# ParBLiSS/kmerhash

Measured on AMD Instinct MI355X. Metric: kmer_inserts_plus_finds_per_sec, higher is better.
Workload: dtype u64

## Files before the change

kmerhash_amd/csrc/kh_kernels.h:

```cpp
#pragma once
#include <hip/hip_runtime.h>
#include <stdint.h>
#include "../../include/kmerhash_amd/kh_hash.h"

#define KH_LB 11
#define KH_L (1u << KH_LB)
#define KH_HS 4096u
#define KH_CHUNK_THREADS 512
#ifndef KH_PART_THREADS
#define KH_PART_THREADS 512
#define KH_PART_MAXPER 4
#endif
#ifndef KH_PART_ITEMS
#define KH_PART_ITEMS 16
#endif
#define KH_PART_TILE (KH_PART_THREADS * KH_PART_ITEMS)
#ifndef KH_PART_STAGE
#define KH_PART_STAGE 4096
#endif
#define KH_NONE 0xFFFFFFFFFFFFFFFFull
#define KH_EMPTY_KEY 0xFFFFFFFFFFFFFFFFull

enum { KHK_RH = 0, KHK_LP = 1 };
enum { KH_FLAG_PROBE_OVERFLOW = 0, KH_FLAG_REGION_OVERFLOW = 1, KH_FLAG_COUNT_OVERFLOW = 2, KH_FLAG_INTERNAL = 3, KH_FLAG_FUSE_INVALID = 4, KH_NFLAGS = 8 };
// ... 777 lines not shown
      const unsigned long long iv = ((unsigned long long)i << 32) | (vbase ? *reinterpret_cast<const uint32_t*>(vbase + i * vstride) : vconst);
      orec[(uint64_t)q * n + pos] = make_ulonglong2(key, iv);
    }
  }
  __syncthreads();
  if (tid == 0) { cursor[q] = (uint64_t)q * n + cnt; starts[q] = (uint64_t)q * n; if (q == 0) starts[gridDim.x] = (uint64_t)gridDim.x * n; }
}

#define KH_SAMPLE_N 65536u
#define KH_SAMPLE_SET (1u << 18)
__global__ void k_sample_dups(const char* __restrict__ kbase, uint32_t kstride, uint64_t n, unsigned long long* __restrict__ set ,
                              uint32_t* __restrict__ dups) {
  const uint32_t i = blockIdx.x * blockDim.x + threadIdx.x;
  if (i >= KH_SAMPLE_N) return;
  const uint64_t pos = (uint64_t)i * (n / KH_SAMPLE_N);
  const unsigned long long key = *reinterpret_cast<const uint64_t*>(kbase + pos * kstride) ^ 0x8000000000000001ull;
  const unsigned long long tag = key ? key : 1ull;
  uint32_t slot = (uint32_t)kh_fmix64(tag) & (KH_SAMPLE_SET - 1);
  for (;;) {
    const unsigned long long cur = atomicCAS(&set[slot], 0ull, tag);
    if (cur == 0ull) break;
    if (cur == tag) { atomicAdd(dups, 1u); break; }
    slot = (slot + 1) & (KH_SAMPLE_SET - 1);
  }
}

__global__ void k_init_cursors2(unsigned long long* __restrict__ cur1, uint64_t n1, uint64_t slot1, unsigned long long* __restrict__ cur2,
                                uint64_t* __restrict__ starts, uint64_t n2, uint64_t slot2, uint32_t* __restrict__ ovf) {
  const uint64_t i = (uint64_t)blockIdx.x * blockDim.x + threadIdx.x;
  if (i < n1) cur1[i] = i * slot1;
  if (i < n2) cur2[i] = i * slot2;
  if (i <= n2) starts[i] = i * slot2;
  if (i == 0) *ovf = 0u;
}
__global__ void k_init_cursors(unsigned long long* __restrict__ cursor, uint64_t* __restrict__ starts, uint64_t n, uint64_t slot) {
  const uint64_t i = (uint64_t)blockIdx.x * blockDim.x + threadIdx.x;
  if (i < n) cursor[i] = i * slot;
  if (starts && i <= n) starts[i] = i * slot;
}

__global__ void k_make_tiles(const uint64_t* __restrict__ segoff, uint32_t nseg, KhTile* __restrict__ tiles, uint32_t* __restrict__ ntiles_out,
                             const unsigned long long* __restrict__ cursor = nullptr, uint64_t slot = 0) {
  __shared__ uint32_t wtot[16];
  __shared__ uint32_t carry_s;
  const uint32_t tid = threadIdx.x, lane = tid & 63, wid = tid >> 6;
  if (tid == 0) carry_s = 0;
  __syncthreads();
  for (uint32_t base = 0; base < nseg; base += 1024) {
    uint32_t s = base + tid;
    uint64_t beg = 0, len = 0;
    if (s < nseg) {
      if (slot) { beg = (uint64_t)s * slot; len = cursor[s] - beg; if (len > slot) len = slot; }
      else { beg = segoff[s]; len = segoff[s + 1] - beg; }
    }
    uint32_t nt = (uint32_t)((len + KH_PART_TILE - 1) / KH_PART_TILE);
    uint32_t incl = nt;
    for (int off = 1; off < 64; off <<= 1) {
      uint32_t o = __shfl_up(incl, off, 64);
      if (lane >= (uint32_t)off) incl += o;
    }
    if (lane == 63) wtot[wid] = incl;
    __syncthreads();
    uint32_t wpre = 0;
    for (uint32_t w = 0; w < wid; ++w) wpre += wtot[w];
    uint32_t carry = carry_s;
    uint32_t first = carry + wpre + incl - nt;
// ... 633 lines not shown
    KhMP v; v.A = KH_MP_NEG; v.n = 0;
#pragma unroll
    for (int j = 0; j < KH_CARRY_ITEMS; ++j) {
      it[j].A = KH_MP_NEG; it[j].n = 0;
      if (c0 + j < nch) { it[j].A = sumA[c0 + j]; it[j].n = sumN[c0 + j]; }
      v = kh_mp_combine(v, it[j]);
    }
    KhMP total;
    KhMP excl = kh_block_scan_mp(v, s_wtot, &total);
    const KhMP carry = s_carry;
    KhMP run = kh_mp_combine(carry, excl);
#pragma unroll
    for (int j = 0; j < KH_CARRY_ITEMS; ++j) {
      if (c0 + j < nch) prefix_tmp[c0 + j] = run;
      run = kh_mp_combine(run, it[j]);
    }
    __syncthreads();
    if (tid == 0) s_carry = kh_mp_combine(carry, total);
    __syncthreads();
  }
  KhMP all = s_carry;
  long long end0 = all.A > all.n ? all.A : all.n;
  long long x0 = end0 - cap;
  if (x0 < 0) x0 = 0;
  for (uint32_t c = tid; c < nch; c += 1024) {
    KhMP p = prefix_tmp[c];
    long long x = x0 + p.n;
    xcarry[c] = p.A > x ? p.A : x;
  }
}

#define KH_SPILL 256
template <int KIND, int HASH>
__global__ __launch_bounds__(KH_CHUNK_THREADS) void k_chunk_place(KhRebuildParams P) {
  __shared__ uint64_t skeys[KH_L + KH_SPILL];
  __shared__ uint32_t svals[KH_L + KH_SPILL];
  __shared__ uint32_t sinfo_w[(KH_L + KH_SPILL) / 4];
  __shared__ uint32_t fill[KH_L];
  __shared__ uint32_t start[KH_L];
  __shared__ uint32_t s_emin;
  __shared__ long long s_pend;
  __shared__ KhMP s_wtot[KH_CHUNK_THREADS / 64];
  uint8_t* sinfo = reinterpret_cast<uint8_t*>(sinfo_w);
  const uint32_t tid = threadIdx.x, c = blockIdx.x;
  const uint32_t Ln = P.New.cap > KH_L ? KH_L : (uint32_t)P.New.cap;
  const uint64_t Sc = (uint64_t)c * Ln, mask_n = P.New.cap - 1;
  const uint32_t empty4 = KIND == KHK_RH ? 0u : 0x40404040u;
  for (uint32_t i = tid; i < KH_L + KH_SPILL; i += KH_CHUNK_THREADS) { skeys[i] = 0; svals[i] = 0; }
  for (uint32_t i = tid; i < (KH_L + KH_SPILL) / 4; i += KH_CHUNK_THREADS) sinfo_w[i] = empty4;
  uint32_t cb[KH_HOMES_PER_THREAD];
  KhMP v; v.A = KH_MP_NEG; v.n = 0;
#pragma unroll
  for (uint32_t j = 0; j < KH_HOMES_PER_THREAD; ++j) {
    uint32_t b = tid * KH_HOMES_PER_THREAD + j;
    cb[j] = b < Ln ? P.homecnt[Sc + b] : 0u;
    if (b < Ln) { KhMP h; h.A = (long long)b + cb[j]; h.n = cb[j]; v = kh_mp_combine(v, h); }
    fill[tid * KH_HOMES_PER_THREAD + j] = 0;
  }
  KhMP excl = kh_block_scan_mp(v, s_wtot, nullptr);
  const long long xr = P.xcarry[c] - (long long)Sc;
  long long p = excl.A > xr + excl.n ? excl.A : xr + excl.n;
#pragma unroll
  for (uint32_t j = 0; j < KH_HOMES_PER_THREAD; ++j) {
    uint32_t b = tid * KH_HOMES_PER_THREAD + j;
    if (b < Ln) {
      long long st = p > (long long)b ? p : (long long)b;
      start[b] = (uint32_t)st;
      p = st + cb[j];
    }
  }
  if (tid == KH_CHUNK_THREADS - 1) s_pend = p;
  __syncthreads();
  auto place = [&](uint64_t key, uint32_t val, uint64_t hn) {
    uint32_t b = (uint32_t)(hn - Sc);
    uint32_t r = atomicAdd(&fill[b], 1u);
    uint32_t prel = start[b] + r;
    uint32_t dist = prel - b;
    uint8_t ib = 0x00;
    if (KIND == KHK_RH) {
      if (dist > 127u) { atomicOr(&P.flags[KH_FLAG_PROBE_OVERFLOW], 1u); dist = 127u; }
      ib = (uint8_t)(0x80u | dist);
    }
    if (prel < KH_L + KH_SPILL) { skeys[prel] = key; svals[prel] = val; sinfo[prel] = ib; }
    else kh_slot_st(P.New.s + ((Sc + prel) & mask_n), key, val, ib);
  };
  kh_for_each_old<KIND, HASH>(P, c, &s_emin, place);
  kh_for_each_new<HASH>(P, c, place);
  __syncthreads();
  long long pend = s_pend;
  if (pend < (long long)Ln) pend = Ln;
  const uint32_t lo = xr > 0 ? (uint32_t)xr : 0u;
  uint32_t hi = pend < (long long)(KH_L + KH_SPILL) ? (uint32_t)pend : (KH_L + KH_SPILL);
  for (uint32_t s0 = lo + tid; s0 < hi; s0 += KH_CHUNK_THREADS) {
    kh_slot_st(P.New.s + ((Sc + s0) & mask_n), skeys[s0], svals[s0], sinfo[s0]);
  }
}

#define KH_XB 127u
#define KH_FSPILL 128u
struct KhFusedParams {
  KhSrcSet src; uint32_t PB;
  KhSlots New; KhSeed seed; int mode;
  unsigned long long* pub;
  uint64_t* ck0; uint32_t* cv0; uint16_t* homecnt0;
  uint32_t* maxidx;
  uint64_t n_total, half_max_load;
  uint64_t base_size;
  unsigned long long* est;
  uint32_t* flags;
  long long poll_limit;
  int nodup;
  KhRebuildParams R;
};

template <int KIND, int HASH, bool MERGE>
__device__ __forceinline__ uint32_t kh_stage_from_table(const KhRebuildParams& R, uint32_t c, uint64_t Sc, unsigned long long* lk,
                                                         unsigned long long* liv, uint32_t* n_staged, uint32_t* scratch) {
  const uint32_t tid = threadIdx.x;
  const uint64_t cap_o = R.Old.cap, mask_o = cap_o - 1, mask_n = R.New.cap - 1;
  if (tid == 0) *n_staged = 0;
  __syncthreads();
  if (cap_o) {
    const uint32_t nch_o = (uint32_t)(cap_o >> KH_LB);
    const uint32_t o = c & (nch_o - 1);
    const bool same = R.New.cap == cap_o;
    const uint64_t S = (uint64_t)o * KH_L;
    uint64_t len = KH_L + 128u;
    if (KIND == KHK_LP) {
      const uint64_t beyond = cap_o - KH_L;
// ... 1234 lines not shown
    if ((late >> k) & 1u) {
      const uint32_t p0 = pj[k] & 0xFFFFu, pc = (pj[k] >> 16) + xr;
      enter(kh_slot_key(w[k]), w[k].z, rank[k] >> 16, p0 > pc ? p0 : pc);
    }
  }
#pragma unroll
  for (uint32_t u = 0; u < 2; ++u) {
    if ((late >> (ROWS + u)) & 1u) {
      const uint32_t i = tid + u * KH_CHUNK_THREADS;
      const uint32_t p0 = pj[ROWS + u] & 0xFFFFu, pc = (pj[ROWS + u] >> 16) + xr;
      enter(rk[i], (uint32_t)riv[i], hbr[u], p0 > pc ? p0 : pc);
    }
  }
  __syncthreads();
  {
    const int tA = total.A > 0 ? total.A : 0;
    int pend = tA > (int)xr + (int)n_c ? tA : (int)xr + (int)n_c;
    if (pend < (int)KH_L) pend = (int)KH_L;
    if (pend > (int)(KH_L + KH_FSPILL)) pend = (int)(KH_L + KH_FSPILL);
#pragma unroll
    for (uint32_t k = 0; k < ROWS; ++k) {
      const int s0 = (int)(base + 64u * k);
      if (k < nrows && s0 >= (int)xr && s0 < pend) {
        const uint32_t ib = iinfo[s0];
        KhSlot* dst = P.New.s + ((Sc + (uint32_t)s0) & mask_n);
        if (ib == 0u) kh_slot_st(dst, 0, 0, kh_empty_info<KHK_RH>());
        else kh_slot_st(dst, ikey[s0], ival[s0], ib);
      }
    }
  }
  (void)n_old;
}

__global__ void k_fused_tail_carry(const unsigned long long* __restrict__ pub, uint32_t nch, long long* __restrict__ xcarry0,
                                   uint64_t* __restrict__ noff0 = nullptr, uint32_t* __restrict__ ncnt0 = nullptr) {
  if (threadIdx.x == 0 && blockIdx.x == 0) {
    xcarry0[0] = (long long)((pub[nch - 1] >> 32) & 0x7FFFFFFFull);
    if (noff0) { noff0[0] = 0; noff0[1] = 0; }
    if (ncnt0) ncnt0[0] = (uint32_t)pub[0];
  }
}

__global__ __launch_bounds__(1024) void k_fused_totals(const unsigned long long* __restrict__ pub, const uint32_t* __restrict__ maxidx, uint32_t nch,
                                                       unsigned long long* __restrict__ totals) {
  __shared__ unsigned long long ws[16];
  __shared__ uint32_t wm[16];
  unsigned long long sum = 0; uint32_t mx = 0;
  for (uint32_t c = blockIdx.x * 1024 + threadIdx.x; c < nch; c += gridDim.x * 1024) { sum += pub[c] & 0xFFFFFFFFull; const uint32_t v = maxidx[c]; mx = v > mx ? v : mx; }
  for (int off = 32; off > 0; off >>= 1) { sum += __shfl_down(sum, off, 64); const uint32_t o = __shfl_down(mx, off, 64); mx = o > mx ? o : mx; }
  if ((threadIdx.x & 63) == 0) { ws[threadIdx.x >> 6] = sum; wm[threadIdx.x >> 6] = mx; }
  __syncthreads();
  if (threadIdx.x == 0) {
    unsigned long long t = 0; uint32_t m = 0;
    for (int w = 0; w < 16; ++w) { t += ws[w]; m = wm[w] > m ? wm[w] : m; }
    if (t) atomicAdd(&totals[0], t);
    if (m) atomicMax(&totals[1], (unsigned long long)m);
  }
}

__global__ void k_disp_hist(const KhSlot* __restrict__ slots, uint64_t cap, unsigned long long* __restrict__ out128) {
  __shared__ uint32_t h[128];
  if (threadIdx.x < 128) h[threadIdx.x] = 0;
  __syncthreads();
  uint64_t i = (uint64_t)blockIdx.x * blockDim.x + threadIdx.x;
  uint64_t stride = (uint64_t)gridDim.x * blockDim.x;
  for (; i < cap; i += stride) { uint32_t b = slots[i].info & 0xFFu; if (b >= 0x80u) atomicAdd(&h[b & 0x7Fu], 1u); }
  __syncthreads();
  if (threadIdx.x < 128 && h[threadIdx.x]) atomicAdd(&out128[threadIdx.x], (unsigned long long)h[threadIdx.x]);
}

template <int KIND>
__global__ void k_unpack_slots(const KhSlot* __restrict__ slots, uint64_t cap, uint64_t* __restrict__ keys, uint32_t* __restrict__ vals,
                               uint8_t* __restrict__ info, uint8_t* __restrict__ flags) {
  uint64_t i = (uint64_t)blockIdx.x * blockDim.x + threadIdx.x;
  uint64_t stride = (uint64_t)gridDim.x * blockDim.x;
  for (; i < cap; i += stride) {
    const uint4 w = kh_slot_ld(slots + i);
    if (keys) keys[i] = kh_slot_key(w);
    if (vals) vals[i] = w.z;
    if (info) info[i] = (uint8_t)(w.w & 0xFFu);
    if (flags) flags[i] = kh_is_occupied<KIND>(w.w & 0xFFu) ? 1 : 0;
  }
}

#define KH_SHARD_THREADS 512
#define KH_SHARD_TILE(KW) (KH_SHARD_THREADS * KhKey<KW>::SHARD_ITEMS)
#define KH_SHARD_MAXR 64
// ... 676 lines not shown
```

kmerhash_amd/csrc/kmerhash_amd.hip:

```cpp
#include "kh_kernels.h"
#include "kh_kernels_wide.h"
#include "kh_kernels_values.h"
#include "kh_kernels_index.h"
#include "kh_kernels_index_wide.h"
#include "kh_kernels_csr.h"
#include "../../include/kmerhash_amd.h"

#include <string>
#include <vector>
#include <cstdio>
#include <cstring>
#include <algorithm>
#include <cmath>
#include <cstdlib>

#include <map>
#include <memory>
#include <mutex>
#include <unordered_map>

#define KH_VERSION_STR "kmerhash_amd 0.1 (gfx950)"

namespace {
struct DevPool {
// ... 47 lines not shown
  P.free_.insert(std::make_pair(it->second, p));
  P.cached += it->second;
}
struct HostPool { std::mutex m; std::vector<uint64_t*> pinned; std::vector<hipEvent_t> events[16]; };
HostPool g_host;
uint64_t* pinned_get() {
  { std::lock_guard<std::mutex> g(g_host.m);
    if (!g_host.pinned.empty()) { uint64_t* p = g_host.pinned.back(); g_host.pinned.pop_back(); return p; } }
  uint64_t* p = nullptr;
  if (hipHostMalloc(reinterpret_cast<void**>(&p), 64 * sizeof(uint64_t)) != hipSuccess) { (void)hipGetLastError(); return nullptr; }
  return p;
}
void pinned_put(uint64_t* p) { if (p) { std::lock_guard<std::mutex> g(g_host.m); g_host.pinned.push_back(p); } }
hipEvent_t event_get(int dev) {
  { std::lock_guard<std::mutex> g(g_host.m);
    auto& v = g_host.events[dev & 15];
    if (!v.empty()) { hipEvent_t e = v.back(); v.pop_back(); return e; } }
  hipEvent_t e = nullptr;
  hipEventCreate(&e);
  return e;
}
void event_put(int dev, hipEvent_t e) { if (e) { std::lock_guard<std::mutex> g(g_host.m); g_host.events[dev & 15].push_back(e); } }
}

namespace {

struct ProfRec { const char* name; hipEvent_t a, b; };

struct Block { char* p; size_t cap; };

}

struct SlackShared { unsigned long long* cur2; uint64_t* starts; uint32_t* ovf; uint64_t slot; };
struct SlotBuf {
  void* p; uint64_t cap;
  SlotBuf() : p(nullptr), cap(0) {}
  SlotBuf(KhSlots s) : p(s.s), cap(s.cap) {}
  SlotBuf(KwSlots s) : p(s.s), cap(s.cap) {}
};
struct kh_table {
  int kind = KHK_RH, hash = 0, device = 0;
  KhSeed seed = KhSeed{0, 0u};
  hipStream_t stream = nullptr;
  float min_lf = 0.f, max_lf = 0.f;
  uint64_t min_load = 0, max_load = 0, lsize = 0;
  uint32_t slot_bytes = sizeof(KhSlot);
  SlotBuf cur, spare;
  std::vector<Block> blocks;
  size_t blk = 0, off = 0;
  uint64_t* hpin = nullptr;
  std::string err;
  struct {
    bool active, fallback, nodup; int mode;
    bool repeatable, slack, rec12;
    SlackShared sh;
    uint64_t n_total, fed, cap_u; uint32_t PB;
    ulonglong2 *tmp, *fin;
    KhSrcSet S;
    uint64_t* stage_k; uint32_t* stage_v;
    const uint64_t* wk[KH_MAX_SRC]; const uint32_t* wv[KH_MAX_SRC]; uint64_t wn[KH_MAX_SRC]; uint32_t wsrc; uint32_t* wcnt;
  } ins = {};
  uint32_t* part_overflow = nullptr;
  double batch_vf = 1.0;
  bool batch_nodup = false;
  bool prof = false;
  std::vector<ProfRec> recs;
  std::vector<std::pair<std::string, std::pair<double, uint64_t> > > prof_acc;
};
struct kh_wtable : kh_table {};

namespace {

inline uint64_t next_pow2(uint64_t x) {
  if (x <= 1) return 1;
  return uint64_t(1) << (64 - __builtin_clzll(x - 1));
}
inline uint64_t threshold(uint64_t buckets, float lf) {
  return static_cast<uint64_t>(static_cast<float>(buckets) * lf);
}
inline uint32_t log2u(uint64_t x) { return 63u - (uint32_t)__builtin_clzll(x); }

kh_status fail(kh_table* t, kh_status s, const std::string& msg) {
  if (t) t->err = msg;
  return s;
}
#define HIPCHK(call)                                                                                   \
  do {                                                                                                 \
    hipError_t e__ = (call);                                                                           \
    if (e__ != hipSuccess)                                                                             \
      return fail(t, e__ == hipErrorOutOfMemory ? KH_ERR_NOMEM : KH_ERR_HIP,                          \
                  std::string(#call) + ": " + hipGetErrorString(e__));                                \
  } while (0)

void arena_reset(kh_table* t) { t->blk = 0; t->off = 0; }
kh_status arena_take(kh_table* t, size_t bytes, void** out) {
// ... 129 lines not shown
  if ((k) == KHK_RH) { constexpr int KIND = KHK_RH; KH_SWITCH_HASH(h, __VA_ARGS__) }  \
  else { constexpr int KIND = KHK_LP; KH_SWITCH_HASH(h, __VA_ARGS__) }

inline uint32_t grid_for(uint64_t n, uint32_t block, uint32_t maxblocks = 256 * 16) {
  uint64_t g = (n + block - 1) / block;
  if (g < 1) g = 1;
  if (g > maxblocks) g = maxblocks;
  return (uint32_t)g;
}

template <typename T>
kh_status stage_in(kh_table* t, const void* p, uint64_t n, kh_mem where, const T** out) {
  if (where == KH_MEM_DEVICE || p == nullptr) { *out = static_cast<const T*>(p); return KH_OK; }
  T* d = nullptr;
  TAKE(d, T, n);
  HIPCHK(hipMemcpyAsync(d, p, sizeof(T) * n, hipMemcpyHostToDevice, t->stream));
  *out = d;
  return KH_OK;
}

inline size_t ws_rebuild(uint64_t cap) { return size_t(cap) * 2 + (cap > KH_L ? (cap >> KH_LB) : 1) * 48 + (size_t(1) << 16); }

struct PreCount { uint16_t* homecnt; long long* sumA; long long* sumN; };

const bool g_disable_fused_rebuild = getenv("KH_DISABLE_FUSED_BUILD") != nullptr || getenv("KH_DISABLE_FUSED_REBUILD") != nullptr;

const long long g_poll_limit = getenv("KH_DEBUG_POLL_LIMIT") ? atoll(getenv("KH_DEBUG_POLL_LIMIT")) : (1ll << 23);
struct FusedRun { unsigned long long* totals; uint32_t* flags; };
const bool g_disable_lean = getenv("KH_DISABLE_LEAN_BUILD") != nullptr;
kh_status launch_fused(kh_table* t, int src, KhFusedParams& F, const KhSlots& nw, uint32_t PB_tail, const char* name, FusedRun* out) {
  const uint32_t nch = (uint32_t)(nw.cap >> KH_LB);
  char* blk; uint32_t* maxidx; uint64_t* ck0; uint32_t* cv0; uint16_t* hc0; long long* xc0; uint64_t* noff0; uint32_t* ncnt0;
  const size_t sz_pub = (size_t)nch * 8, sz_ctl = sz_pub + 256, sz_all = sz_ctl + (size_t)nch * 4;
  TAKE(blk, char, sz_all);
  maxidx = reinterpret_cast<uint32_t*>(blk + sz_ctl);
  TAKE(ck0, uint64_t, KH_DD_M); TAKE(cv0, uint32_t, KH_DD_M); TAKE(hc0, uint16_t, KH_L); TAKE(xc0, long long, 1);
  TAKE(noff0, uint64_t, 2); TAKE(ncnt0, uint32_t, 1);
  HIPCHK(hipMemsetAsync(blk, 0, sz_all, t->stream));
  F.New = nw; F.seed = t->seed;
  F.pub = reinterpret_cast<unsigned long long*>(blk);
  unsigned long long* totals = reinterpret_cast<unsigned long long*>(blk + sz_pub);
  F.maxidx = maxidx; F.ck0 = ck0; F.cv0 = cv0; F.homecnt0 = hc0;
  F.est = reinterpret_cast<unsigned long long*>(blk + sz_pub + 32);
  F.flags = reinterpret_cast<uint32_t*>(blk + sz_pub + 64);
  F.poll_limit = g_poll_limit;
  F.R.New = nw; F.R.seed = t->seed; F.R.flags = F.flags;
  { Launch L(t, name);
    const double mean_c = (double)F.n_total / (double)nch;
    const bool lean_fits = mean_c + 5.0 * std::sqrt(mean_c) < (double)KH_LEAN_M;
    if (src == 0 && F.nodup && F.src.rec12 == 1 && F.src.n == 1 && lean_fits && !g_disable_lean) { KH_SWITCH_KIND_HASH(t->kind, t->hash, hipLaunchKernelGGL((k_build_lean<KIND, HASH>), dim3(nch), dim3(KH_CHUNK_THREADS), 0, t->stream, F)); }
    else if (src == 0) { KH_SWITCH_KIND_HASH(t->kind, t->hash, hipLaunchKernelGGL((k_build_fused<KIND, HASH, 0>), dim3(nch), dim3(KH_CHUNK_THREADS), 0, t->stream, F)); }
    else if (src == 1) { KH_SWITCH_KIND_HASH(t->kind, t->hash, hipLaunchKernelGGL((k_build_fused<KIND, HASH, 1>), dim3(nch), dim3(KH_CHUNK_THREADS), 0, t->stream, F)); }
    else if (src == 3) { KH_SWITCH_HASH(t->hash, hipLaunchKernelGGL((k_build_fused<KHK_RH, HASH, 3>), dim3(nch), dim3(KH_CHUNK_THREADS), 0, t->stream, F)); }
    else if (src == 4) { KH_SWITCH_HASH(t->hash, hipLaunchKernelGGL((k_erase_stream<HASH>), dim3(nch), dim3(KH_CHUNK_THREADS), 0, t->stream, F)); }
    else if (src == 5) { KH_SWITCH_HASH(t->hash, hipLaunchKernelGGL((k_insert_stream<HASH>), dim3(nch), dim3(KH_CHUNK_THREADS), 0, t->stream, F)); }
    else { KH_SWITCH_KIND_HASH(t->kind, t->hash, hipLaunchKernelGGL((k_build_fused<KIND, HASH, 2>), dim3(nch), dim3(KH_CHUNK_THREADS), 0, t->stream, F)); } }
  { Launch L(t, "k_fused_totals");
    hipLaunchKernelGGL(k_fused_totals, dim3(std::max<uint32_t>(1u, std::min<uint32_t>(64u, nch / 1024u))), dim3(1024), 0, t->stream, F.pub, maxidx, nch, totals); }
  {
    Launch L(t, "k_fused_tail");
    hipLaunchKernelGGL(k_fused_tail_carry, dim3(1), dim3(64), 0, t->stream, F.pub, nch, xc0, noff0, ncnt0);
    KhRebuildParams T0;
    memset(&T0, 0, sizeof(T0));
    T0.Old = kNoSlots; T0.New = nw; T0.ck = ck0; T0.cv = cv0; T0.noff = noff0; T0.ncnt = ncnt0; T0.PB = PB_tail;
    T0.seed = t->seed; T0.homecnt = hc0; T0.xcarry = xc0; T0.flags = F.flags;
    KH_SWITCH_KIND_HASH(t->kind, t->hash, hipLaunchKernelGGL((k_chunk_place<KIND, HASH>), dim3(1), dim3(KH_CHUNK_THREADS), 0, t->stream, T0));
  }
  HIPCHK(hipGetLastError());
  HIPCHK(hipMemcpyAsync(t->hpin, blk + sz_pub, 128, hipMemcpyDeviceToHost, t->stream));
  t->hpin[30] = 0;
  if (t->part_overflow) HIPCHK(hipMemcpyAsync(t->hpin + 30, t->part_overflow, 4, hipMemcpyDeviceToHost, t->stream));
  HIPCHK(hipStreamSynchronize(t->stream));
  out->totals = totals; out->flags = F.flags;
  return KH_OK;
}

const char* const kProbeOverflowText = "Robin Hood probe distance would exceed 127 (7-bit info field, hashmap_robinhood.hpp:142-144,556)";
const char* const kDedupOverflowText = "internal: de-duplication set overflow";
kh_status flags_status(kh_table* t, const uint32_t* f) {
  if (f[KH_FLAG_PROBE_OVERFLOW]) return fail(t, KH_ERR_PROBE_OVERFLOW, kProbeOverflowText);
  if (f[KH_FLAG_REGION_OVERFLOW]) return fail(t, KH_ERR_PROBE_OVERFLOW, "cluster longer than one chunk (2048 slots) without an empty slot");
  if (f[KH_FLAG_COUNT_OVERFLOW]) return fail(t, KH_ERR_PROBE_OVERFLOW, "more than 65535 keys share one home bucket");
  if (f[KH_FLAG_INTERNAL]) return fail(t, KH_ERR_HIP, kDedupOverflowText);
  return KH_OK;
}

struct Narrow {
  typedef KhSlots Slots; typedef KhRebuildParams Params;
  static Slots view(const SlotBuf& b) { return narrow(b); }
  static void set_seed(Params& P, const kh_table* t) { P.seed = t->seed; }
  static void count(kh_table* t, uint32_t nch, const Params& P) {
    Launch L(t, "k_chunk_count");
    KH_SWITCH_KIND_HASH(t->kind, t->hash, hipLaunchKernelGGL((k_chunk_count<KIND, HASH>), dim3(nch), dim3(KH_CHUNK_THREADS), 0, t->stream, P));
  }
  static void place(kh_table* t, uint32_t nch, const Params& P) {
    Launch L(t, "k_chunk_place");
    KH_SWITCH_KIND_HASH(t->kind, t->hash, hipLaunchKernelGGL((k_chunk_place<KIND, HASH>), dim3(nch), dim3(KH_CHUNK_THREADS), 0, t->stream, P));
  }
};
struct Wide {
  typedef KwSlots Slots; typedef KwRebuildParams Params;
  static Slots view(const SlotBuf& b) { return wide(b); }
  static void set_seed(Params& P, const kh_table* t) { P.seed = t->seed.s; }
  static void count(kh_table* t, uint32_t nch, const Params& P) {
// ... 94 lines not shown
    n = rh_rehash_capacity(n, t->lsize, t->max_lf);
    if (n == t->cur.cap) return KH_OK;
  } else if (t->lsize > n) {
    return fail(t, KH_ERR_FULL, "ERROR: did not find any place to insert.  should not have happend (hashmap_linearprobe.hpp:408)");
  }
  { kh_status ps = arena_prepare(t, ws_rebuild(n)); if (ps != KH_OK) return ps; }
  return rebuild(t, n, nullptr, nullptr, nullptr, nullptr, 0, false, t->lsize);
}
kh_status do_reserve(kh_table* t, uint64_t n) {
  if (n > t->max_load) return do_rehash(t, static_cast<uint64_t>(static_cast<float>(n) / t->max_lf));
  return KH_OK;
}

struct Partitioned {
  ulonglong2* rec;
  uint64_t* part_off;
  uint32_t PB, nparts;
  ulonglong2* spare;
  uint64_t slot;
  const unsigned long long* cursor;
  uint32_t* overflow;
  int rec12;
};
inline uint64_t slack_slot(double mean, double vf = 1.0) { return (uint64_t)(mean + 7.0 * std::sqrt(mean * vf) + 16.0); }
const bool g_disable_slack = getenv("KH_DISABLE_SLACK_PARTITION") != nullptr;
const int g_xcd_swizzle = getenv("KH_DISABLE_XCD_SWIZZLE") ? 0 : 1;
inline uint64_t part_buffer_records(uint64_t n, uint32_t PB, bool allow_slack, double vf = 1.0) {
  if (!allow_slack || g_disable_slack || PB <= 11 || n < (uint64_t(256) << PB)) return n;
  return (slack_slot((double)n / (double)(uint64_t(1) << PB), vf) << PB) + KH_PART_TILE;
}

kh_status partition_batch(kh_table* t, const char* kbase, uint32_t kstride, const char* vbase, uint32_t vstride,
                          uint32_t vconst, uint64_t n, uint64_t idx_base, uint32_t PB, ulonglong2* tmp, ulonglong2* fin, Partitioned& out,
                          bool allow_slack = false, int rec12 = 0, const SlackShared* shared = nullptr, bool force_slack = false, double vf = 1.0) {
  const uint32_t nparts = 1u << PB;
  out.slot = 0; out.cursor = nullptr; out.overflow = nullptr; out.rec12 = 0;
  if (shared || force_slack || part_buffer_records(n, PB, allow_slack, vf) != n) {
    const uint32_t B1 = (PB + 1) / 2, B2 = PB - B1, nb1 = 1u << B1, nb2 = 1u << B2;
    const uint64_t slot = shared ? shared->slot : slack_slot((double)n / (double)nparts, vf);
    const uint64_t slot1 = shared ? slack_slot((double)n / (double)nb1) : slot * nb2;
    unsigned long long *cur1, *cur2; uint64_t* starts; uint32_t* ovf;
    TAKE(cur1, unsigned long long, nb1);
    if (shared) { cur2 = shared->cur2; starts = shared->starts; ovf = shared->ovf; }
    else { TAKE(cur2, unsigned long long, nparts); TAKE(starts, uint64_t, (size_t)nparts + 1); TAKE(ovf, uint32_t, 1); }
    const double mean1 = (double)n / (double)nb1;
    const uint64_t fill_cap = std::min<uint64_t>(slot1, (uint64_t)(mean1 + 9.0 * std::sqrt(mean1 * vf) + 16.0));
    const uint32_t tps = (uint32_t)((fill_cap + KH_PART_TILE - 1) / KH_PART_TILE);
    const uint32_t max_tiles = nb1 * tps;
    if (shared) hipLaunchKernelGGL(k_init_cursors, dim3((nb1 + 255) / 256), dim3(256), 0, t->stream, cur1, (uint64_t*)nullptr, (uint64_t)nb1, slot1);
    else hipLaunchKernelGGL(k_init_cursors2, dim3((nparts + 256) / 256), dim3(256), 0, t->stream, cur1, (uint64_t)nb1, slot1, cur2, starts, (uint64_t)nparts, slot, ovf);
    KhPartParams P;
    memset(&P, 0, sizeof(P));
    P.idx_base = idx_base;
    P.xcd_swizzle = g_xcd_swizzle;
    P.kbase = kbase; P.kstride = kstride; P.vbase = vbase; P.vstride = vstride; P.vconst = vconst; P.n = n;
    P.ntiles = (uint32_t)((n + KH_PART_TILE - 1) / KH_PART_TILE);
    P.seed = t->seed; P.PB = PB; P.shift = B2; P.nb = nb1; P.cursor = cur1; P.orec = tmp; P.slot = slot1; P.overflow = ovf; P.dump = slot1 * nb1;
    { Launch L(t, "k_part_scatter");
      if (rec12 == 1) { KH_SWITCH_HASH(t->hash, hipLaunchKernelGGL((k_part_scatter<HASH, 1>), dim3(P.ntiles), dim3(KH_PART_THREADS), ((nb1 + 1u) & ~1u) * 8 + nb1 * 8, t->stream, P)); }
      else if (rec12 == 2) { KH_SWITCH_HASH(t->hash, hipLaunchKernelGGL((k_part_scatter<HASH, 2>), dim3(P.ntiles), dim3(KH_PART_THREADS), ((nb1 + 1u) & ~1u) * 8 + nb1 * 8, t->stream, P)); }
      else { KH_SWITCH_HASH(t->hash, hipLaunchKernelGGL((k_part_scatter<HASH, 0>), dim3(P.ntiles), dim3(KH_PART_THREADS), ((nb1 + 1u) & ~1u) * 8 + nb1 * 8, t->stream, P)); } }
    KhPartParams Q = P;
    Q.kbase = nullptr; Q.kstride = 0; Q.vbase = nullptr; Q.vstride = 0; Q.rec_in = tmp;
    Q.tiles = nullptr; Q.ntiles_dev = nullptr; Q.ntiles = max_tiles; Q.slot_in = slot1; Q.cur_in = cur1; Q.tps = tps;
    Q.shift = 0; Q.nb = nb2; Q.cursor = cur2; Q.orec = fin; Q.slot = slot; Q.dump = slot * nparts;
    { Launch L(t, "k_part_scatter");
      if (rec12 == 1) { KH_SWITCH_HASH(t->hash, hipLaunchKernelGGL((k_part_scatter<HASH, 1>), dim3(max_tiles), dim3(KH_PART_THREADS), ((nb2 + 1u) & ~1u) * 8 + nb2 * 8, t->stream, Q)); }
      else if (rec12 == 2) { KH_SWITCH_HASH(t->hash, hipLaunchKernelGGL((k_part_scatter<HASH, 2>), dim3(max_tiles), dim3(KH_PART_THREADS), ((nb2 + 1u) & ~1u) * 8 + nb2 * 8, t->stream, Q)); }
      else { KH_SWITCH_HASH(t->hash, hipLaunchKernelGGL((k_part_scatter<HASH, 0>), dim3(max_tiles), dim3(KH_PART_THREADS), ((nb2 + 1u) & ~1u) * 8 + nb2 * 8, t->stream, Q)); } }
    HIPCHK(hipGetLastError());
    out.rec = fin; out.part_off = starts; out.PB = PB; out.nparts = nparts; out.spare = tmp;
    out.slot = slot; out.cursor = cur2; out.overflow = ovf; out.rec12 = rec12;
    return KH_OK;
  }
  if (rec12 == 1) return fail(t, KH_ERR_HIP, "internal: record kind not available with exact offsets");
  ulonglong2* ar = nullptr; ulonglong2* br = fin;
  const uint32_t B1 = PB <= 11 ? PB : (PB + 1) / 2, B2 = PB - B1;
  const uint32_t nb1 = 1u << B1, nb2 = 1u << B2;
  ar = B2 ? tmp : fin;
  uint32_t* counts1; uint64_t* off1; unsigned long long* cur1;
  TAKE(counts1, uint32_t, nb1); TAKE(off1, uint64_t, nb1 + 1); TAKE(cur1, unsigned long long, nb1);
  KhPartParams P;
// ... 90 lines not shown
inline bool ins_flags_ok(unsigned flags) {
  if (flags & ~(unsigned)(KH_INS_REDUCE_PLUS | KH_INS_REPEATABLE | KH_INS_REDUCE_OP_MASK)) return false;
  return (flags & KH_INS_REDUCE_PLUS) || !(flags & KH_INS_REDUCE_OP_MASK);
}
inline int ins_flags_mode(unsigned flags) {
  return (flags & KH_INS_REDUCE_PLUS) ? INS_PLUS + (int)((flags & KH_INS_REDUCE_OP_MASK) >> KH_INS_REDUCE_OP_SHIFT) : INS_FIRST;
}
const uint64_t g_max_pass = getenv("KH_MAX_PASS_RECORDS") ? std::max<uint64_t>(1024, std::min<uint64_t>(strtoull(getenv("KH_MAX_PASS_RECORDS"), nullptr, 10), 0xFFFFFFF0ull))
                                                          : (uint64_t(1) << 30);
bool g_disable_fused = getenv("KH_DISABLE_FUSED_BUILD") != nullptr;

const kh_status KH_RETRY_EXACT = static_cast<kh_status>(100);
kh_status insert_finish(kh_table* t, KhSrcSet S, uint64_t n, uint32_t PB, uint64_t cap_u, int mode, uint64_t forced_cap,
                        ulonglong2* spare, uint64_t* n_new_out, uint64_t list_cap = 0);

inline bool fused_build_applies(const kh_table* t, uint64_t cap_u, uint32_t PB) {
  return t->lsize == 0 && cap_u >= 2 * (uint64_t)KH_L && t->max_lf <= 0.9f && PB == log2u(cap_u >> KH_LB) && !g_disable_fused;
}
inline bool nodup_build_applies(const kh_table* t, uint64_t cap_u, uint32_t PB, int mode) {
  return fused_build_applies(t, cap_u, PB) && t->batch_nodup && (mode == INS_FIRST || mode == INS_PLUS) && !getenv("KH_DISABLE_NODUP");
}

kh_status insert_core(kh_table* t, const char* kbase, uint32_t kstride, const char* vbase, uint32_t vstride,
                      uint64_t n, int mode, uint64_t forced_cap, uint64_t* n_new_out) {
  *n_new_out = 0;
  if (n == 0) return KH_OK;
  const uint64_t cap_u = forced_cap ? forced_cap : capacity_after(t, t->cur.cap, t->lsize, n, n, n - 1);
  const uint32_t PB = cap_u > KH_L ? log2u(cap_u >> KH_LB) : 0u;
  if (PB > 22) return fail(t, KH_ERR_UNSUPPORTED, "batch would need more than 2^22 partitions");
  const size_t keep_blk = t->blk, keep_off = t->off;
  int first_attempt = 0;
  bool dup_heavy = false;
  double vf = 1.0;
  if (part_buffer_records(n, PB, true) != n) {
    unsigned long long* sset; uint32_t* dups;
    TAKE(sset, unsigned long long, KH_SAMPLE_SET); TAKE(dups, uint32_t, 1);
    HIPCHK(hipMemsetAsync(sset, 0, sizeof(unsigned long long) * KH_SAMPLE_SET, t->stream));
    HIPCHK(hipMemsetAsync(dups, 0, 4, t->stream));
    { Launch L(t, "k_sample_dups");
      hipLaunchKernelGGL(k_sample_dups, dim3(KH_SAMPLE_N / 256), dim3(256), 0, t->stream, kbase, kstride, n, sset, dups); }
    HIPCHK(hipMemcpyAsync(t->hpin + 31, dups, 4, hipMemcpyDeviceToHost, t->stream));
    HIPCHK(hipStreamSynchronize(t->stream));
    const uint32_t dsample = (uint32_t)t->hpin[31];
    if (dsample >= 1u) {
      dup_heavy = true;
      const double d_ub = (double)dsample + 3.0 * std::sqrt((double)dsample) + 3.0;
      const double f = 1.0 + 2.0 * (double)n * d_ub / ((double)KH_SAMPLE_N * (double)KH_SAMPLE_N);
      const double mean = (double)n / (double)(uint64_t(1) << PB);
      if (!getenv("KH_DISABLE_DUP_SLACK") && (double)slack_slot(mean, f) <= 2.0 * mean) vf = f;
      else first_attempt = 1;
    }
    t->batch_nodup = dsample == 0u;
    t->blk = keep_blk; t->off = keep_off;
  } else first_attempt = 1;
  for (int attempt = first_attempt; attempt < 2; ++attempt) {
    const bool slack = attempt == 0;
    const uint64_t m = part_buffer_records(n, PB, slack, vf);
    if (!slack && attempt == 1) { t->blk = keep_blk; t->off = keep_off; }
    const bool rec12 = slack && t->batch_nodup && nodup_build_applies(t, cap_u, PB, mode);
    const bool rec8 = !rec12 && dup_heavy && mode == INS_PLUS && vbase == nullptr && !getenv("KH_DISABLE_REC8");
    const int kind = rec12 ? 1 : rec8 ? 2 : 0;
    ulonglong2 *tmp, *fin, *spare;
    { char *a, *b; const size_t rb = kind == 1 ? sizeof(KhRec12) : kind == 2 ? sizeof(KhRec8) : sizeof(ulonglong2);
      TAKE(a, char, m * rb); TAKE(b, char, m * rb);
      tmp = reinterpret_cast<ulonglong2*>(a); fin = reinterpret_cast<ulonglong2*>(b); spare = tmp;
      if (kind == 2) { char* c; TAKE(c, char, m * 12); spare = reinterpret_cast<ulonglong2*>(c); } }
    Partitioned R;
    kh_status st = partition_batch(t, kbase, kstride, vbase, vstride, mode == INS_PLUS ? 1u : 0u, n, 0, PB, tmp, fin, R, slack, kind, nullptr, false, vf);
    if (st != KH_OK) return st;
    KhSrcSet S;
    memset(&S, 0, sizeof(S));
    S.rec[0] = R.rec; S.off[0] = R.part_off; S.n = 1; S.merged_off = R.part_off; S.slot[0] = R.slot; S.cur[0] = R.cursor;
    S.rec12 = (uint32_t)R.rec12;
    t->part_overflow = R.overflow; t->batch_vf = vf;
    st = insert_finish(t, S, n, PB, cap_u, mode, forced_cap, spare, n_new_out, m);
    t->part_overflow = nullptr; t->batch_nodup = false; t->batch_vf = 1.0;
    if (st != KH_RETRY_EXACT) return st;
  }
  return fail(t, KH_ERR_HIP, "internal: exact partition reported a slot overflow");
}

kh_status insert_finish(kh_table* t, KhSrcSet S, uint64_t n, uint32_t PB, uint64_t cap_u, int mode, uint64_t forced_cap,
                        ulonglong2* spare, uint64_t* n_new_out, uint64_t list_cap) {
  *n_new_out = 0;
  if (list_cap < n) list_cap = n;
  kh_status st = KH_OK;
  const uint32_t nparts = 1u << PB;
  struct { uint32_t nparts; } R; R.nparts = nparts;
  if (fused_build_applies(t, cap_u, PB) && one_launch_mode(mode) && S.rec12 != 2 && !(t->batch_vf >= 2.0)) {
    const uint32_t nch = (uint32_t)(cap_u >> KH_LB);
    KhSlots nw;
    st = fresh_slots(t, cap_u, nw);
    if (st != KH_OK) return st;
    KhFusedParams F;
    memset(&F, 0, sizeof(F));
    F.src = S; F.PB = PB;
    F.mode = mode == INS_PLUS ? KH_DEDUP_PLUS : KH_DEDUP_FIRST;
    F.base_size = 0;
    F.n_total = n;
    F.nodup = nodup_build_applies(t, cap_u, PB, mode) ? 1 : 0;
    F.half_max_load = (cap_u >> 1) >= t->cur.cap ? threshold(cap_u >> 1, t->max_lf) : 0;
    FusedRun run;
    { kh_status fs = launch_fused(t, 0, F, nw, PB, "k_build_fused", &run); if (fs != KH_OK) return fs; }
    if (t->part_overflow && (uint32_t)t->hpin[30]) { retire_slots(t, nw); return KH_RETRY_EXACT; }
    unsigned long long* totals = run.totals;
    const uint64_t fd = t->hpin[0];
    const uint64_t flast = (mode == INS_PLUS || S.rec12) ? n - 1 : (t->hpin[1] ? t->hpin[1] - 1 : 0);
    const uint32_t* ff = reinterpret_cast<const uint32_t*>(reinterpret_cast<const char*>(t->hpin) + 64);
    bool bad = S.rec12 && fd != n;
// ... 569 lines not shown
    retire_slots(t, nw);
    t->blk = keep_blk; t->off = keep_off;
  }
  unsigned long long* cnt;
  TAKE(cnt, unsigned long long, 1);
  HIPCHK(hipMemsetAsync(cnt, 0, 8, t->stream));
  { Launch L(t, "k_erase_mark");
    KH_SWITCH_KIND_HASH(t->kind, t->hash, hipLaunchKernelGGL((k_erase_mark<KIND, HASH>), dim3(grid_for(n, KH_Q_THREADS * KH_Q_ITEMS, 2048)), dim3(KH_Q_THREADS), 0, t->stream, narrow(t->cur), q, n, t->seed, cnt)); }
  HIPCHK(hipGetLastError());
  HIPCHK(hipMemcpyAsync(t->hpin, cnt, 8, hipMemcpyDeviceToHost, t->stream));
  HIPCHK(hipStreamSynchronize(t->stream));
  const uint64_t ne = t->hpin[0];
  if (ne && t->kind == KHK_RH) {
    st = rebuild(t, t->cur.cap, nullptr, nullptr, nullptr, nullptr, 0, true, t->lsize - ne);
    if (st != KH_OK) {
      hipLaunchKernelGGL(k_clear_marks, dim3(grid_for(t->cur.cap, 256)), dim3(256), 0, t->stream, narrow(t->cur));
      hipStreamSynchronize(t->stream);
      return st;
    }
  }
  t->lsize -= ne;
  *n_erased = ne;
  return KH_OK;
}

bool valid(const kh_table* t) { return t != nullptr; }
kh_status table_init(kh_table* t, int kind, int hash, uint64_t seed, uint64_t capacity, float min_lf, float max_lf, int device) {
  t->kind = kind; t->hash = hash; t->device = device; t->seed = KhSeed{seed, 0u};
  t->min_lf = min_lf; t->max_lf = max_lf;
  const uint64_t cap = next_pow2(capacity);
  if (alloc_slots(t, cap, t->cur) != KH_OK) return KH_ERR_NOMEM;
  t->hpin = pinned_get();
  if (!t->hpin) { free_slots(t, t->cur); return KH_ERR_NOMEM; }
  if (fill_empty(t, t->cur) != KH_OK || hipStreamSynchronize(t->stream) != hipSuccess) { free_slots(t, t->cur); pinned_put(t->hpin); return KH_ERR_HIP; }
  t->min_load = threshold(cap, min_lf);
  t->max_load = threshold(cap, max_lf);
  return KH_OK;
}
void table_release(kh_table* t) {
  if (!t) return;
  hipSetDevice(t->device);
  hipStreamSynchronize(t->stream);
  for (auto& r : t->recs) { event_put(t->device, r.a); event_put(t->device, r.b); }
  free_slots(t, t->cur); free_slots(t, t->spare);
  for (auto& b : t->blocks) pool_free(t->device, b.p);
  pinned_put(t->hpin);
}

}

extern "C" {

const char* kh_version(void) { return KH_VERSION_STR; }

kh_status kh_release_cached_memory(int device) {
  if (device < 0 || device >= 16) return KH_ERR_INVALID;
  if (hipSetDevice(device) != hipSuccess) return KH_ERR_HIP;
  hipDeviceSynchronize();
  pool_trim(device);
  return KH_OK;
}

kh_status kh_create(kh_table** out, kh_kind kind, uint32_t key_bytes, uint32_t val_bytes, kh_hash hash, uint64_t seed,
                    uint64_t capacity, float min_lf, float max_lf, int device) {
  if (!out) return KH_ERR_INVALID;
  *out = nullptr;
  if (key_bytes != 8 || val_bytes != 4) return KH_ERR_UNSUPPORTED;
// ... 2106 lines not shown
```

Before: 44.10 billion.

## Merge init memsets and epilogue kernels to cut launches and copies

Folds the sample-set memset, dups memset, cursor initialisation and fused-control-block zeroing into a single bulk-init kernel issued before dup sampling, then reuses those pre-initialised buffers in partition and fused build. Merges the totals, tail-carry and single-chunk tail placement kernels into one epilogue kernel, which also copies the partition overflow flag so the host needs one 256-byte readback instead of two copies. Also drops a stream sync at table init. The aim is fewer kernel launches, memsets and small copies per batch, at the cost of more buffer-reuse bookkeeping, where a mismatch between the preallocated parameters and the recomputed slot sizes falls back to the old path.

```diff
diff --git a/kmerhash_amd/csrc/kh_kernels.h b/kmerhash_amd/csrc/kh_kernels.h
--- a/kmerhash_amd/csrc/kh_kernels.h
+++ b/kmerhash_amd/csrc/kh_kernels.h
@@ -833,6 +833,19 @@
   if (i < n2) cur2[i] = i * slot2;
   if (i <= n2) starts[i] = i * slot2;
   if (i == 0) *ovf = 0u;
+}
+__global__ void k_bulk_init(uint4* __restrict__ set16, uint64_t nset16, uint32_t* __restrict__ dups, unsigned long long* __restrict__ cur1, uint64_t n1, uint64_t slot1,
+                            unsigned long long* __restrict__ cur2, uint64_t* __restrict__ starts, uint64_t n2, uint64_t slot2, uint32_t* __restrict__ ovf,
+                            uint4* __restrict__ z16, uint64_t nz16) {
+  const uint64_t step = (uint64_t)gridDim.x * blockDim.x;
+  for (uint64_t i = (uint64_t)blockIdx.x * blockDim.x + threadIdx.x; i < nset16 || i <= n2 || i < nz16; i += step) {
+    if (i < nset16) set16[i] = make_uint4(0u, 0u, 0u, 0u);
+    if (i < nz16) z16[i] = make_uint4(0u, 0u, 0u, 0u);
+    if (i < n1) cur1[i] = i * slot1;
+    if (i < n2) cur2[i] = i * slot2;
+    if (i <= n2) starts[i] = i * slot2;
+    if (i == 0) { *ovf = 0u; *dups = 0u; }
+  }
 }
 __global__ void k_init_cursors(unsigned long long* __restrict__ cursor, uint64_t* __restrict__ starts, uint64_t n, uint64_t slot) {
   const uint64_t i = (uint64_t)blockIdx.x * blockDim.x + threadIdx.x;
@@ -1532,7 +1545,7 @@
 
 #define KH_SPILL 256
 template <int KIND, int HASH>
-__global__ __launch_bounds__(KH_CHUNK_THREADS) void k_chunk_place(KhRebuildParams P) {
+__device__ __forceinline__ void kh_chunk_place_body(const KhRebuildParams& P, const uint32_t c) {
   __shared__ uint64_t skeys[KH_L + KH_SPILL];
   __shared__ uint32_t svals[KH_L + KH_SPILL];
   __shared__ uint32_t sinfo_w[(KH_L + KH_SPILL) / 4];
@@ -1542,7 +1555,7 @@
   __shared__ long long s_pend;
   __shared__ KhMP s_wtot[KH_CHUNK_THREADS / 64];
   uint8_t* sinfo = reinterpret_cast<uint8_t*>(sinfo_w);
-  const uint32_t tid = threadIdx.x, c = blockIdx.x;
+  const uint32_t tid = threadIdx.x;
   const uint32_t Ln = P.New.cap > KH_L ? KH_L : (uint32_t)P.New.cap;
   const uint64_t Sc = (uint64_t)c * Ln, mask_n = P.New.cap - 1;
   const uint32_t empty4 = KIND == KHK_RH ? 0u : 0x40404040u;
@@ -1595,6 +1608,8 @@
     kh_slot_st(P.New.s + ((Sc + s0) & mask_n), skeys[s0], svals[s0], sinfo[s0]);
   }
 }
+template <int KIND, int HASH>
+__global__ __launch_bounds__(KH_CHUNK_THREADS) void k_chunk_place(KhRebuildParams P) { kh_chunk_place_body<KIND, HASH>(P, blockIdx.x); }
 
 #define KH_XB 127u
 #define KH_FSPILL 128u
@@ -2895,27 +2910,34 @@
   (void)n_old;
 }
 
-__global__ void k_fused_tail_carry(const unsigned long long* __restrict__ pub, uint32_t nch, long long* __restrict__ xcarry0,
-                                   uint64_t* __restrict__ noff0 = nullptr, uint32_t* __restrict__ ncnt0 = nullptr) {
-  if (threadIdx.x == 0 && blockIdx.x == 0) {
-    xcarry0[0] = (long long)((pub[nch - 1] >> 32) & 0x7FFFFFFFull);
-    if (noff0) { noff0[0] = 0; noff0[1] = 0; }
-    if (ncnt0) ncnt0[0] = (uint32_t)pub[0];
-  }
-}
-
-__global__ __launch_bounds__(1024) void k_fused_totals(const unsigned long long* __restrict__ pub, const uint32_t* __restrict__ maxidx, uint32_t nch,
-                                                       unsigned long long* __restrict__ totals) {
-  __shared__ unsigned long long ws[16];
-  __shared__ uint32_t wm[16];
+template <int KIND, int HASH>
+__global__ __launch_bounds__(KH_CHUNK_THREADS) void k_fused_epilogue(KhRebuildParams T0, const unsigned long long* __restrict__ pub, const uint32_t* __restrict__ maxidx,
+                                                                     uint32_t nch, unsigned long long* __restrict__ totals, long long* xcarry0, uint64_t* noff0,
+                                                                     uint32_t* ncnt0, const uint32_t* __restrict__ ovf, uint32_t* __restrict__ ovf_out) {
+  if (blockIdx.x == 0) {
+    if (threadIdx.x == 0) {
+      xcarry0[0] = (long long)((pub[nch - 1] >> 32) & 0x7FFFFFFFull);
+      noff0[0] = 0; noff0[1] = 0;
+      ncnt0[0] = (uint32_t)pub[0];
+      ovf_out[0] = ovf ? ovf[0] : 0u;
+    }
+    __threadfence();
+    __syncthreads();
+    kh_chunk_place_body<KIND, HASH>(T0, 0u);
+    return;
+  }
+  __shared__ unsigned long long ws[KH_CHUNK_THREADS / 64];
+  __shared__ uint32_t wm[KH_CHUNK_THREADS / 64];
   unsigned long long sum = 0; uint32_t mx = 0;
-  for (uint32_t c = blockIdx.x * 1024 + threadIdx.x; c < nch; c += gridDim.x * 1024) { sum += pub[c] & 0xFFFFFFFFull; const uint32_t v = maxidx[c]; mx = v > mx ? v : mx; }
+  for (uint32_t c = (blockIdx.x - 1) * KH_CHUNK_THREADS + threadIdx.x; c < nch; c += (gridDim.x - 1) * KH_CHUNK_THREADS) {
+    sum += pub[c] & 0xFFFFFFFFull; const uint32_t v = maxidx[c]; mx = v > mx ? v : mx;
+  }
   for (int off = 32; off > 0; off >>= 1) { sum += __shfl_down(sum, off, 64); const uint32_t o = __shfl_down(mx, off, 64); mx = o > mx ? o : mx; }
   if ((threadIdx.x & 63) == 0) { ws[threadIdx.x >> 6] = sum; wm[threadIdx.x >> 6] = mx; }
   __syncthreads();
   if (threadIdx.x == 0) {
     unsigned long long t = 0; uint32_t m = 0;
-    for (int w = 0; w < 16; ++w) { t += ws[w]; m = wm[w] > m ? wm[w] : m; }
+    for (int w = 0; w < KH_CHUNK_THREADS / 64; ++w) { t += ws[w]; m = wm[w] > m ? wm[w] : m; }
     if (t) atomicAdd(&totals[0], t);
     if (m) atomicMax(&totals[1], (unsigned long long)m);
   }
diff --git a/kmerhash_amd/csrc/kmerhash_amd.hip b/kmerhash_amd/csrc/kmerhash_amd.hip
--- a/kmerhash_amd/csrc/kmerhash_amd.hip
+++ b/kmerhash_amd/csrc/kmerhash_amd.hip
@@ -103,6 +103,7 @@
 }
 
 struct SlackShared { unsigned long long* cur2; uint64_t* starts; uint32_t* ovf; uint64_t slot; };
+struct SlackPre { unsigned long long *cur1, *cur2; uint64_t* starts; uint32_t* ovf; uint64_t slot, slot1; uint32_t PB; };
 struct SlotBuf {
   void* p; uint64_t cap;
   SlotBuf() : p(nullptr), cap(0) {}
@@ -132,6 +133,7 @@
     const uint64_t* wk[KH_MAX_SRC]; const uint32_t* wv[KH_MAX_SRC]; uint64_t wn[KH_MAX_SRC]; uint32_t wsrc; uint32_t* wcnt;
   } ins = {};
   uint32_t* part_overflow = nullptr;
+  char* pre_ctl = nullptr; size_t pre_ctl_bytes = 0;
   double batch_vf = 1.0;
   bool batch_nodup = false;
   bool prof = false;
@@ -327,11 +329,13 @@
   const uint32_t nch = (uint32_t)(nw.cap >> KH_LB);
   char* blk; uint32_t* maxidx; uint64_t* ck0; uint32_t* cv0; uint16_t* hc0; long long* xc0; uint64_t* noff0; uint32_t* ncnt0;
   const size_t sz_pub = (size_t)nch * 8, sz_ctl = sz_pub + 256, sz_all = sz_ctl + (size_t)nch * 4;
-  TAKE(blk, char, sz_all);
+  const bool prezeroed = t->pre_ctl && t->pre_ctl_bytes == sz_all;
+  if (prezeroed) blk = t->pre_ctl; else TAKE(blk, char, sz_all);
+  t->pre_ctl = nullptr; t->pre_ctl_bytes = 0;
   maxidx = reinterpret_cast<uint32_t*>(blk + sz_ctl);
   TAKE(ck0, uint64_t, KH_DD_M); TAKE(cv0, uint32_t, KH_DD_M); TAKE(hc0, uint16_t, KH_L); TAKE(xc0, long long, 1);
   TAKE(noff0, uint64_t, 2); TAKE(ncnt0, uint32_t, 1);
-  HIPCHK(hipMemsetAsync(blk, 0, sz_all, t->stream));
+  if (!prezeroed) HIPCHK(hipMemsetAsync(blk, 0, sz_all, t->stream));
   F.New = nw; F.seed = t->seed;
   F.pub = reinterpret_cast<unsigned long long*>(blk);
   unsigned long long* totals = reinterpret_cast<unsigned long long*>(blk + sz_pub);
@@ -350,21 +354,19 @@
     else if (src == 4) { KH_SWITCH_HASH(t->hash, hipLaunchKernelGGL((k_erase_stream<HASH>), dim3(nch), dim3(KH_CHUNK_THREADS), 0, t->stream, F)); }
     else if (src == 5) { KH_SWITCH_HASH(t->hash, hipLaunchKernelGGL((k_insert_stream<HASH>), dim3(nch), dim3(KH_CHUNK_THREADS), 0, t->stream, F)); }
     else { KH_SWITCH_KIND_HASH(t->kind, t->hash, hipLaunchKernelGGL((k_build_fused<KIND, HASH, 2>), dim3(nch), dim3(KH_CHUNK_THREADS), 0, t->stream, F)); } }
-  { Launch L(t, "k_fused_totals");
-    hipLaunchKernelGGL(k_fused_totals, dim3(std::max<uint32_t>(1u, std::min<uint32_t>(64u, nch / 1024u))), dim3(1024), 0, t->stream, F.pub, maxidx, nch, totals); }
   {
     Launch L(t, "k_fused_tail");
-    hipLaunchKernelGGL(k_fused_tail_carry, dim3(1), dim3(64), 0, t->stream, F.pub, nch, xc0, noff0, ncnt0);
     KhRebuildParams T0;
     memset(&T0, 0, sizeof(T0));
     T0.Old = kNoSlots; T0.New = nw; T0.ck = ck0; T0.cv = cv0; T0.noff = noff0; T0.ncnt = ncnt0; T0.PB = PB_tail;
     T0.seed = t->seed; T0.homecnt = hc0; T0.xcarry = xc0; T0.flags = F.flags;
-    KH_SWITCH_KIND_HASH(t->kind, t->hash, hipLaunchKernelGGL((k_chunk_place<KIND, HASH>), dim3(1), dim3(KH_CHUNK_THREADS), 0, t->stream, T0));
+    const uint32_t g_tot = std::max<uint32_t>(1u, std::min<uint32_t>(64u, nch / 1024u));
+    KH_SWITCH_KIND_HASH(t->kind, t->hash, hipLaunchKernelGGL((k_fused_epilogue<KIND, HASH>), dim3(1 + g_tot), dim3(KH_CHUNK_THREADS), 0, t->stream, T0, (const unsigned long long*)F.pub,
+                                                             (const uint32_t*)maxidx, nch, totals, xc0, noff0, ncnt0, (const uint32_t*)t->part_overflow,
+                                                             reinterpret_cast<uint32_t*>(blk + sz_pub + 240)));
   }
   HIPCHK(hipGetLastError());
-  HIPCHK(hipMemcpyAsync(t->hpin, blk + sz_pub, 128, hipMemcpyDeviceToHost, t->stream));
-  t->hpin[30] = 0;
-  if (t->part_overflow) HIPCHK(hipMemcpyAsync(t->hpin + 30, t->part_overflow, 4, hipMemcpyDeviceToHost, t->stream));
+  HIPCHK(hipMemcpyAsync(t->hpin, blk + sz_pub, 256, hipMemcpyDeviceToHost, t->stream));
   HIPCHK(hipStreamSynchronize(t->stream));
   out->totals = totals; out->flags = F.flags;
   return KH_OK;
@@ -525,7 +527,8 @@
 
 kh_status partition_batch(kh_table* t, const char* kbase, uint32_t kstride, const char* vbase, uint32_t vstride,
                           uint32_t vconst, uint64_t n, uint64_t idx_base, uint32_t PB, ulonglong2* tmp, ulonglong2* fin, Partitioned& out,
-                          bool allow_slack = false, int rec12 = 0, const SlackShared* shared = nullptr, bool force_slack = false, double vf = 1.0) {
+                          bool allow_slack = false, int rec12 = 0, const SlackShared* shared = nullptr, bool force_slack = false, double vf = 1.0,
+                          const SlackPre* pre = nullptr) {
   const uint32_t nparts = 1u << PB;
   out.slot = 0; out.cursor = nullptr; out.overflow = nullptr; out.rec12 = 0;
   if (shared || force_slack || part_buffer_records(n, PB, allow_slack, vf) != n) {
@@ -533,14 +536,19 @@
     const uint64_t slot = shared ? shared->slot : slack_slot((double)n / (double)nparts, vf);
     const uint64_t slot1 = shared ? slack_slot((double)n / (double)nb1) : slot * nb2;
     unsigned long long *cur1, *cur2; uint64_t* starts; uint32_t* ovf;
-    TAKE(cur1, unsigned long long, nb1);
-    if (shared) { cur2 = shared->cur2; starts = shared->starts; ovf = shared->ovf; }
-    else { TAKE(cur2, unsigned long long, nparts); TAKE(starts, uint64_t, (size_t)nparts + 1); TAKE(ovf, uint32_t, 1); }
+    const bool preset = pre && !shared && pre->PB == PB && pre->slot == slot && pre->slot1 == slot1;
+    if (preset) { cur1 = pre->cur1; cur2 = pre->cur2; starts = pre->starts; ovf = pre->ovf; }
+    else {
+      TAKE(cur1, unsigned long long, nb1);
+      if (shared) { cur2 = shared->cur2; starts = shared->starts; ovf = shared->ovf; }
+      else { TAKE(cur2, unsigned long long, nparts); TAKE(starts, uint64_t, (size_t)nparts + 1); TAKE(ovf, uint32_t, 1); }
+    }
     const double mean1 = (double)n / (double)nb1;
     const uint64_t fill_cap = std::min<uint64_t>(slot1, (uint64_t)(mean1 + 9.0 * std::sqrt(mean1 * vf) + 16.0));
     const uint32_t tps = (uint32_t)((fill_cap + KH_PART_TILE - 1) / KH_PART_TILE);
     const uint32_t max_tiles = nb1 * tps;
-    if (shared) hipLaunchKernelGGL(k_init_cursors, dim3((nb1 + 255) / 256), dim3(256), 0, t->stream, cur1, (uint64_t*)nullptr, (uint64_t)nb1, slot1);
+    if (preset) {}
+    else if (shared) hipLaunchKernelGGL(k_init_cursors, dim3((nb1 + 255) / 256), dim3(256), 0, t->stream, cur1, (uint64_t*)nullptr, (uint64_t)nb1, slot1);
     else hipLaunchKernelGGL(k_init_cursors2, dim3((nparts + 256) / 256), dim3(256), 0, t->stream, cur1, (uint64_t)nb1, slot1, cur2, starts, (uint64_t)nparts, slot, ovf);
     KhPartParams P;
     memset(&P, 0, sizeof(P));
@@ -697,11 +705,27 @@
   int first_attempt = 0;
   bool dup_heavy = false;
   double vf = 1.0;
+  SlackPre pre; memset(&pre, 0, sizeof(pre));
+  bool have_pre = false;
+  t->pre_ctl = nullptr; t->pre_ctl_bytes = 0;
   if (part_buffer_records(n, PB, true) != n) {
+    const uint32_t nparts0 = 1u << PB, nb1_0 = 1u << ((PB + 1) / 2);
+    pre.PB = PB; pre.slot = slack_slot((double)n / (double)nparts0); pre.slot1 = pre.slot * (nparts0 / nb1_0);
+    TAKE(pre.cur1, unsigned long long, nb1_0); TAKE(pre.cur2, unsigned long long, nparts0); TAKE(pre.starts, uint64_t, (size_t)nparts0 + 1); TAKE(pre.ovf, uint32_t, 1);
+    char* zctl = nullptr; size_t zbytes = 0;
+    if (fused_build_applies(t, cap_u, PB) && one_launch_mode(mode)) {
+      const size_t nch0 = (size_t)(cap_u >> KH_LB);
+      zbytes = nch0 * 8 + 256 + nch0 * 4;
+      TAKE(zctl, char, zbytes);
+    }
+    have_pre = true;
+    const size_t keep2_blk = t->blk, keep2_off = t->off;
     unsigned long long* sset; uint32_t* dups;
     TAKE(sset, unsigned long long, KH_SAMPLE_SET); TAKE(dups, uint32_t, 1);
-    HIPCHK(hipMemsetAsync(sset, 0, sizeof(unsigned long long) * KH_SAMPLE_SET, t->stream));
-    HIPCHK(hipMemsetAsync(dups, 0, 4, t->stream));
+    { const uint64_t nset16 = (uint64_t)KH_SAMPLE_SET / 2, nz16 = (uint64_t)(zbytes + 15) / 16;
+      const uint64_t most = std::max<uint64_t>(std::max<uint64_t>(nset16, nz16), (uint64_t)nparts0 + 1);
+      hipLaunchKernelGGL(k_bulk_init, dim3(grid_for(most, 256, 1024)), dim3(256), 0, t->stream, reinterpret_cast<uint4*>(sset), nset16, dups, pre.cur1, (uint64_t)nb1_0, pre.slot1,
+                         pre.cur2, pre.starts, (uint64_t)nparts0, pre.slot, pre.ovf, reinterpret_cast<uint4*>(zctl), nz16); }
     { Launch L(t, "k_sample_dups");
       hipLaunchKernelGGL(k_sample_dups, dim3(KH_SAMPLE_N / 256), dim3(256), 0, t->stream, kbase, kstride, n, sset, dups); }
     HIPCHK(hipMemcpyAsync(t->hpin + 31, dups, 4, hipMemcpyDeviceToHost, t->stream));
@@ -716,12 +740,13 @@
       else first_attempt = 1;
     }
     t->batch_nodup = dsample == 0u;
-    t->blk = keep_blk; t->off = keep_off;
+    t->blk = keep2_blk; t->off = keep2_off;
+    t->pre_ctl = zctl; t->pre_ctl_bytes = zbytes;
   } else first_attempt = 1;
   for (int attempt = first_attempt; attempt < 2; ++attempt) {
     const bool slack = attempt == 0;
     const uint64_t m = part_buffer_records(n, PB, slack, vf);
-    if (!slack && attempt == 1) { t->blk = keep_blk; t->off = keep_off; }
+    if (!slack && attempt == 1) { t->blk = keep_blk; t->off = keep_off; have_pre = false; t->pre_ctl = nullptr; t->pre_ctl_bytes = 0; }
     const bool rec12 = slack && t->batch_nodup && nodup_build_applies(t, cap_u, PB, mode);
     const bool rec8 = !rec12 && dup_heavy && mode == INS_PLUS && vbase == nullptr && !getenv("KH_DISABLE_REC8");
     const int kind = rec12 ? 1 : rec8 ? 2 : 0;
@@ -731,7 +756,8 @@
       tmp = reinterpret_cast<ulonglong2*>(a); fin = reinterpret_cast<ulonglong2*>(b); spare = tmp;
       if (kind == 2) { char* c; TAKE(c, char, m * 12); spare = reinterpret_cast<ulonglong2*>(c); } }
     Partitioned R;
-    kh_status st = partition_batch(t, kbase, kstride, vbase, vstride, mode == INS_PLUS ? 1u : 0u, n, 0, PB, tmp, fin, R, slack, kind, nullptr, false, vf);
+    kh_status st = partition_batch(t, kbase, kstride, vbase, vstride, mode == INS_PLUS ? 1u : 0u, n, 0, PB, tmp, fin, R, slack, kind, nullptr, false, vf, have_pre && slack ? &pre : nullptr);
+    have_pre = false;
     if (st != KH_OK) return st;
     KhSrcSet S;
     memset(&S, 0, sizeof(S));
@@ -740,6 +766,7 @@
     t->part_overflow = R.overflow; t->batch_vf = vf;
     st = insert_finish(t, S, n, PB, cap_u, mode, forced_cap, spare, n_new_out, m);
     t->part_overflow = nullptr; t->batch_nodup = false; t->batch_vf = 1.0;
+    t->pre_ctl = nullptr; t->pre_ctl_bytes = 0;
     if (st != KH_RETRY_EXACT) return st;
   }
   return fail(t, KH_ERR_HIP, "internal: exact partition reported a slot overflow");
@@ -1375,7 +1402,7 @@
   if (alloc_slots(t, cap, t->cur) != KH_OK) return KH_ERR_NOMEM;
   t->hpin = pinned_get();
   if (!t->hpin) { free_slots(t, t->cur); return KH_ERR_NOMEM; }
-  if (fill_empty(t, t->cur) != KH_OK || hipStreamSynchronize(t->stream) != hipSuccess) { free_slots(t, t->cur); pinned_put(t->hpin); return KH_ERR_HIP; }
+  if (fill_empty(t, t->cur) != KH_OK) { free_slots(t, t->cur); pinned_put(t->hpin); return KH_ERR_HIP; }
   t->min_load = threshold(cap, min_lf);
   t->max_load = threshold(cap, max_lf);
   return KH_OK;
```

After: 44.38 billion (median of 6 runs). No clear change (+0.6%).
